# HpWang-whu/RoReg

Measured on AMD Instinct MI355X. Metric: pair-registrations/sec, higher is better.
Workload: dtype f32 (every f32 operand enters the fp16 matrix cores as hi + lo fp16 under a per-keypoint power-of-two block scale: <= 22 significant bits relative to a CONSERVATIVE per-keypoint bound -- measured on the extractor: the bound sits 2^2..2^6 above the keypoint's true coefficient maximum (config.f16x2_sc

## Files before the change

include/roreg_hip.h:

```cpp
#ifndef ROREG_HIP_H
#define ROREG_HIP_H

#include <stdint.h>
#include <stddef.h>

#ifdef __cplusplus
extern "C" {
#endif

#define ROREG_ABI_VERSION 6
int roreg_abi_version(void);
const char *roreg_last_error(void);

int roreg_set_group_tables(const int32_t *P_host, const int32_t *Nei_host, const double *R_host);

size_t roreg_group_conv_packed_size(int Cin, int Cout, int KS);
int roreg_group_conv_pack_weights(const float *W_host , int Cin, int Cout, int KS,
                                  float *wpack_host );
size_t roreg_group_conv_workspace_size(int B, int Cin, int Cout, int Lin, int Lout, int KS);
int roreg_group_conv(const float *x, const float *wpack, const float *bias,
                     const float *bn_scale, const float *bn_shift, const float *residual,
                     float *out, const int32_t *gather,
                     int B, int Cin, int Cout, int Lin, int Lout, int KS,
                     float *workspace, size_t workspace_floats, void *stream);
// ... 186 lines not shown
int roreg_sinkhorn_batch2(const float *src_final, const float *tgt_final, const int32_t *seg_src, const int32_t *seg_tgt,
                          const int32_t *seg_src_host, const int32_t *seg_tgt_host, const float *consts, int n_seg, float alpha, int iters,
                          int64_t *matches0, int64_t *matches1, float *mscores0, float *mscores1, float *ws, size_t ws_floats,
                          int recompute, void *stream);
size_t roreg_sinkhorn_batch3_workspace_size(int n_seg, int max_m, int max_n, long long total_m, long long total_n, int recompute, int want_Z);
int roreg_sinkhorn_batch3(const float *src_final, const float *tgt_final, const int32_t *seg_src, const int32_t *seg_tgt,
                          const int32_t *seg_src_host, const int32_t *seg_tgt_host, const float *consts, int n_seg, float alpha, int iters,
                          int64_t *matches0, int64_t *matches1, float *mscores0, float *mscores1, float *ws, size_t ws_floats,
                          int recompute, float *Z_out, void *stream);
int roreg_write_files(const char *const *paths, const void *const *headers, const int32_t *header_len, const void *const *data,
                      const int64_t *nbytes, int n, int n_threads);
int roreg_yohoc_draw_many(const uint32_t *seeds, int n_pairs, const int64_t *anchors, const int64_t *offsets, int max_iter, int max_tries,
                          int64_t *rows_out, int32_t *n_hyp_out, double *giveup_out, int n_threads);
size_t roreg_mlp_head_workspace(int L, int n_seg, int C1);
int roreg_mlp_head(const float *x, const float *pos, const float *table, const int64_t *idx, const float *conf, int m, int k, int L, int Cin,
                   const float *W1, const float *b1, int C1, const float *Wr, const float *br, float *h, float *y, const int32_t *seg_off,
                   int n_seg, int mult, float eps, float *mean_rstd, double *ws, void *stream);
int roreg_sinkhorn_early_exit(int on);
int roreg_sinkhorn_iteration_stats(long long *iterations, long long *pairs, int reset, void *stream);

int roreg_set_fourier_tables(const float *F_host);
size_t roreg_irrep_gemm_tiles(int O, int B, int32_t *tiles_host);
size_t roreg_irrep_gemm_tiles_m(int O, int B, int tile_m , int32_t *tiles_host);
int roreg_irrep_gemm(const float *const *X, float *const *Out, const float *const *Add, const float *const *Wpack, int C, int O, int B,
                     const int32_t *tiles_dev, int n_tiles, void *stream);
int roreg_irrep_gemm_split(const float *const *X, float *const *Out, const float *const *Add, const void *const *Wsplit, int C, int O, int B,
                           const int32_t *tiles_dev, int n_tiles, void *stream);
int roreg_irrep_gemm_f16x2(const float *const *X, float *const *Out, const float *const *Add, const void *const *Wsplit2,
                           const float *x_bound_dev, int w_exp, const float *next_u_dev, const float *next_v_dev, float *out_bound_dev,
                           int C, int O, int B, const int32_t *tiles_dev, int n_tiles,
                           int tile_m ,
                           int x_planes , void *stream);
int roreg_gemm_persistent(int on);
int roreg_row_bound(const void *x_spatial, int x_bf16 , const float *bn_scale, const float *bn_shift,
                    float *bound_out, int B, int C, void *stream);
int roreg_ft_nonlin(const float *Xin , const float *x_spatial, const float *bias,
                    const float *bias2, const float *bn_scale, const float *bn_shift, const float *resid_spatial,
                    float *Xout , float *out_spatial ,
                    const int32_t *g_map ,
                    int Lout , int Lvalid,
                    int B, int C, int split ,
                    const float *out_bound ,
                    float *out_rowmax ,
                    int spatial_bf16 ,
                    int out_planes ,
                    void *stream);
int roreg_ft_nonlin_packed(const float *Xin, const float *bias, const float *bn_scale, const float *bn_shift, uint32_t *out_words,
                           const int32_t *g_map, int Lout, int Lvalid, int B, int C, const float *out_bound, float *raw_col, int raw_g,
                           void *stream);

int roreg_profile_enable(int on);
int roreg_profile_read(int slot, double *total_ms, int *launches);

#ifdef __cplusplus
}
#endif
#endif
```

roreg_amd/_abi.py:

```python
import ctypes
from ctypes import c_int, c_void_p, c_size_t, c_double, c_float, c_char_p

import numpy as np

ABI_VERSION = 6

_P = c_void_p
PROTOTYPES = {
    'roreg_abi_version': (c_int, []),
    'roreg_last_error': (c_char_p, []),
    'roreg_set_group_tables': (c_int, [_P, _P, _P]),
    'roreg_group_conv_packed_size': (c_size_t, [c_int, c_int, c_int]),
    'roreg_group_conv_pack_weights': (c_int, [_P, c_int, c_int, c_int, _P]),
    'roreg_group_conv_workspace_size': (c_size_t, [c_int, c_int, c_int, c_int, c_int, c_int]),
    'roreg_group_conv': (c_int, [_P, _P, _P, _P, _P, _P, _P, _P, c_int, c_int, c_int, c_int, c_int, c_int, _P, c_size_t, _P]),
    'roreg_group_conv_split': (c_int, [_P, _P, _P, _P, _P, _P, _P, _P, c_int, c_int, c_int, c_int, c_int, c_int, c_int, _P]),
    'roreg_group_conv_f16x2': (c_int, [_P, _P, c_int, _P, _P, _P, c_float, c_float, _P, _P, _P, _P, _P, c_int, c_int, c_int, c_int, c_int, c_int, c_int, _P]),
    'roreg_group_conv_f16x2_packed': (c_int, [_P, _P, c_int, _P, _P, _P, _P, _P, _P, c_int, c_int, c_int, c_int, c_int, c_int, c_int, _P]),
    'roreg_dense_f16x2': (c_int, [_P, _P, c_int, _P, _P, _P, c_float, c_float, _P, _P, c_int, _P, _P, c_int, c_int, c_int, _P]),
    'roreg_dense_split': (c_int, [_P, _P, _P, _P, _P, _P, c_int, _P, c_int, c_int, c_int, _P]),
    'roreg_gf_finalize': (c_int, [_P, _P, c_int, _P, c_int, _P]),
    'roreg_det_score': (c_int, [_P, _P, c_int, _P]),
    'roreg_inv_descriptor': (c_int, [_P, c_int, _P, c_int, _P]),
    'roreg_nn_search': (c_int, [_P, _P, c_int, _P, _P, c_int, c_int, _P, _P, _P, _P]),
# ... 18 lines not shown
    'roreg_quat_to_trans': (c_int, [_P, _P, _P, _P, _P, _P, c_int, _P, _P, _P]),
    'roreg_ransac_score': (c_int, [_P, _P, _P, c_int, c_int, _P, _P, c_int, c_double, _P, _P, _P, _P]),
    'roreg_refine': (c_int, [_P, _P, _P, c_int, c_int, _P, c_int, _P, _P, _P, c_double, _P, _P, _P]),
    'roreg_lt_prepare_batch': (c_int, [_P, c_int, c_int, c_int, _P, _P, _P, _P, _P, _P]),
    'roreg_lt_finish_batch': (c_int, [_P, c_int, c_int, _P, _P, _P, _P]),
    'roreg_ransac_batch_workspace': (c_size_t, [c_int, ctypes.c_longlong, c_int]),
    'roreg_ransac_batch': (c_int, [_P, c_int, ctypes.c_longlong, c_int, c_int, c_double, c_int, _P, _P, _P, _P, _P, _P, c_size_t, _P]),
    'roreg_refine_batch': (c_int, [_P, _P, c_int, ctypes.c_longlong, _P, ctypes.c_double, c_int, _P, _P, _P, _P]),
    'roreg_yohoc_draw': (c_int, [_P, ctypes.c_longlong, _P, _P, c_int, c_int, _P, _P, _P, _P]),
    'roreg_gather_rows_batch': (c_int, [_P, c_int, c_int, c_int, _P]),
    'roreg_gather_rows_f64': (c_int, [_P, _P, c_int, c_int, _P, _P]),
    'roreg_group_corr': (c_int, [_P, _P, _P, _P, c_int, c_int, _P, _P, _P]),
    'roreg_topk_dot_workspace_size': (c_size_t, [c_int, c_int, c_int]),
    'roreg_topk_dot': (c_int, [_P, c_int, _P, c_int, c_int, _P, _P, _P, c_size_t, _P, _P, c_int, c_int, c_int, _P]),
    'roreg_context_colmax': (c_int, [_P, c_int, _P, c_int, c_int, _P, _P, _P]),
    'roreg_sinkhorn_batch_workspace_size': (c_size_t, [c_int, c_int, c_int, ctypes.c_longlong, ctypes.c_longlong]),
    'roreg_sinkhorn_batch_consts': (c_int, [_P, _P, c_int, _P]),
    'roreg_sinkhorn_batch': (c_int, [_P, _P, _P, _P, _P, _P, _P, c_int, c_float, c_int, _P, _P, _P, _P, _P, c_size_t, _P]),
    'roreg_sinkhorn_batch2_workspace_size': (c_size_t, [c_int, c_int, c_int, ctypes.c_longlong, ctypes.c_longlong]),
    'roreg_sinkhorn_batch2': (c_int, [_P, _P, _P, _P, _P, _P, _P, c_int, c_float, c_int, _P, _P, _P, _P, _P, c_size_t, c_int, _P]),
    'roreg_sinkhorn_batch3_workspace_size': (c_size_t, [c_int, c_int, c_int, ctypes.c_longlong, ctypes.c_longlong, c_int, c_int]),
    'roreg_sinkhorn_batch3': (c_int, [_P, _P, _P, _P, _P, _P, _P, c_int, c_float, c_int, _P, _P, _P, _P, _P, c_size_t, c_int, _P, _P]),
    'roreg_write_files': (c_int, [_P, _P, _P, _P, _P, c_int, c_int]),
    'roreg_yohoc_draw_many': (c_int, [_P, c_int, _P, _P, c_int, c_int, _P, _P, _P, c_int]),
    'roreg_mlp_head_workspace': (c_size_t, [c_int, c_int, c_int]),
    'roreg_mlp_head': (c_int, [_P, _P, _P, _P, _P, c_int, c_int, c_int, c_int, _P, _P, c_int, _P, _P, _P, _P, _P, c_int, c_int, c_float, _P, _P, _P]),
    'roreg_sinkhorn_early_exit': (c_int, [c_int]),
    'roreg_sinkhorn_iteration_stats': (c_int, [_P, _P, c_int, _P]),
    'roreg_linear': (c_int, [_P, c_int, c_int, _P, _P, c_int, _P, _P]),
    'roreg_linear_mfma': (c_int, [_P, c_int, c_int, _P, _P, c_int, _P, _P]),
    'roreg_linear_path': (c_int, [c_int]),
    'roreg_linear_cat3': (c_int, [_P, _P, _P, _P, c_int, c_int, _P, _P, c_int, _P, _P]),
    'roreg_gemm_persistent': (c_int, [c_int]),
    'roreg_instnorm_stats': (c_int, [_P, c_int, c_int, c_float, _P, _P, _P, c_int, c_int, _P]),
    'roreg_mlp_tail': (c_int, [_P, c_int, c_int, _P, _P, _P, _P, _P, c_int, c_int, _P]),
    'roreg_mlp_tail_mfma': (c_int, [_P, c_int, c_int, _P, _P, _P, _P, _P, c_int, c_int, _P]),
    'roreg_knn_attention': (c_int, [_P, _P, _P, _P, c_int, c_int, c_int, c_int, _P, _P]),
    'roreg_rm_elementwise': (c_int, [c_int, _P, _P, _P, _P, c_int, c_int, c_int, _P, _P, _P]),
    'roreg_sinkhorn_workspace_size': (c_size_t, [c_int, c_int]),
    'roreg_sinkhorn': (c_int, [_P, c_int, _P, c_int, c_float, c_int, _P, _P, _P, _P, _P, _P, c_size_t, _P]),
    'roreg_profile_enable': (c_int, [c_int]),
    'roreg_profile_read': (c_int, [c_int, _P, _P]),
    'roreg_set_fourier_tables': (c_int, [_P]),
    'roreg_mt_shuffle_prefix': (c_int, [_P, c_int, _P, c_int, c_int, _P, c_int]),
    'roreg_mt_stream_shuffle_prefix': (c_int, [_P, _P, _P, c_int, c_int, _P]),
    'roreg_irrep_gemm_tiles': (c_size_t, [c_int, c_int, _P]),
    'roreg_irrep_gemm_tiles_m': (c_size_t, [c_int, c_int, c_int, _P]),
    'roreg_irrep_gemm': (c_int, [_P, _P, _P, _P, c_int, c_int, c_int, _P, c_int, _P]),
    'roreg_irrep_gemm_split': (c_int, [_P, _P, _P, _P, c_int, c_int, c_int, _P, c_int, _P]),
    'roreg_irrep_gemm_f16x2': (c_int, [_P, _P, _P, _P, _P, c_int, _P, _P, _P, c_int, c_int, c_int, _P, c_int, c_int, c_int, _P]),
    'roreg_row_bound': (c_int, [_P, c_int, _P, _P, _P, c_int, c_int, _P]),
    'roreg_ft_nonlin': (c_int, [_P, _P, _P, _P, _P, _P, _P, _P, _P, _P, c_int, c_int, c_int, c_int, c_int, _P, _P, c_int, c_int, _P]),
    'roreg_ft_nonlin_packed': (c_int, [_P, _P, _P, _P, _P, _P, c_int, c_int, c_int, c_int, _P, _P, c_int, _P]),
}


_RANSAC_TASK = np.dtype([('keys0', np.uint64), ('keys1', np.uint64), ('matches', np.uint64), ('w', np.uint64), ('Trans', np.uint64),
                         ('hyp_rows', np.uint64), ('M', np.int32), ('H', np.int32), ('koff', np.int64)])

_MATCH_TASK = np.dtype([('desc0', np.uint64), ('desc1', np.uint64), ('rows0', np.uint64), ('rows1', np.uint64), ('m0', np.int32), ('m1', np.int32)])

_GATHER_TASK = np.dtype([('src', np.uint64), ('rows', np.uint64), ('dst', np.uint64), ('n', np.int32), ('pad', np.int32)])

_LT_TASK = np.dtype([('before0', np.uint64), ('before1', np.uint64), ('after0', np.uint64), ('after1', np.uint64), ('keys0', np.uint64),
                     ('keys1', np.uint64), ('matches', np.uint64), ('sel', np.uint64), ('n', np.int32), ('pad', np.int32), ('off', np.int64),
                     ('coef0', np.uint64), ('coef1', np.uint64)])
# ... 1 lines not shown
```

roreg_amd/_hip_fourier.py:

```python
import os
from ctypes import c_void_p

import numpy as np
import torch

from . import hip as _core
from .hip import HipError, _check, _feat, _ptr, _stream, lib

__all__ = ['DenseSplitLayer', 'IRREP_DIMS', 'IRREP_OFFSETS', '_bf16_split3', '_keypoint_of_columns', '_ptr_array', '_res_ptr', '_tile_cache', 'bf16_split3_pack', 'bound_exp', 'coef_pitch', 'coef_size', 'coef_views', 'dense_split', 'ensure_fourier', 'f16_scale_exp', 'f16_split2_pack', 'ft_nonlin', 'ft_nonlin_packed', 'gemm_persistent', 'group_conv_split_pack', 'irrep_gemm', 'next_bound', 'next_bound_spatial', 'pack_coefs_f16x2', 'row_bound', 'unpack_coefs_f16x2', 'words_to_planes']


_fourier_ready = False
IRREP_DIMS = (1, 3, 3, 4, 5)
IRREP_OFFSETS = (0, 1, 10, 19, 35, 60)


def ensure_fourier():
    global _fourier_ready
    if not _fourier_ready:
        from .fourier import group_fourier
        F = np.ascontiguousarray(group_fourier().F, np.float32)
        _check(lib().roreg_set_fourier_tables(F.ctypes.data), 'roreg_set_fourier_tables')
        _fourier_ready = True


def _ptr_array(views):
    arr = (c_void_p * 5)(*[c_void_p(v.data_ptr()) for v in views])
    return arr


def coef_pitch(B):
    return (int(B) + 31) // 32 * 32


def coef_size(C, B):
    return 60 * C * coef_pitch(B)


def coef_views(buf, C, B):
    Bp = coef_pitch(B)
    return [buf[IRREP_OFFSETS[r] * C * Bp:IRREP_OFFSETS[r + 1] * C * Bp].view(IRREP_DIMS[r] * C, IRREP_DIMS[r] * Bp) for r in range(5)]

# ... 27 lines not shown
        nu = nv = None
        if next_bound is not None:
            nu, nv = next_bound
            if nu.numel() != O or nv.numel() != O:
                raise HipError('irrep_gemm: next_bound must hold one (u, v) per output channel')
            bound_out = torch.zeros(Bp, dtype=torch.float32, device=X_buf.device)
        _check(lib().roreg_irrep_gemm_f16x2(_ptr_array(xv), _ptr_array(ov), av, _ptr_array(wl), _ptr(x_bound, torch.float32), int(w_exp),
                                            _ptr(nu, torch.float32), _ptr(nv, torch.float32), _ptr(bound_out), C, O, Bp,
                                            _ptr(t, torch.int32), int(t.shape[0]), tile_m, (int(x_planes) if x_planes in (1, 2) and x_planes is not True else (2 if _core.MFMA16 else 1)) if x_planes else 0, _stream()), 'roreg_irrep_gemm_f16x2')
    elif split is not None:
        _check(lib().roreg_irrep_gemm_split(_ptr_array(xv), _ptr_array(ov), av, _ptr_array(split), C, O, Bp, _ptr(t, torch.int32), int(t.shape[0]),
                                            _stream()), 'roreg_irrep_gemm_split')
    else:
        _check(lib().roreg_irrep_gemm(_ptr_array(xv), _ptr_array(ov), av, _ptr_array(Wpacks), C, O, Bp, _ptr(t, torch.int32), int(t.shape[0]), _stream()),
               'roreg_irrep_gemm')
    if _core.PROFILE is not None:
        e1.record(); _core.PROFILE.append((('irrep_gemm_f16x2' if f16x2 is not None else 'irrep_gemm_split' if split is not None else 'irrep_gemm', Bp, C, O), e0, e1))
    return (out, bound_out) if next_bound is not None else out


class gemm_persistent:

    def __init__(self, on=True):
        self.on = int(on)

    def __enter__(self):
        self.prev = lib().roreg_gemm_persistent(self.on)

    def __exit__(self, *exc):
        lib().roreg_gemm_persistent(self.prev)
        return False


def row_bound(x, bn=None):
    B, C = int(x.shape[0]), int(x.shape[1])
    out = torch.empty(coef_pitch(B), dtype=torch.float32, device=x.device)
    scale, shift = bn if bn is not None else (None, None)
    xp, bf = _feat(x)
    _check(lib().roreg_row_bound(xp, bf, _ptr(scale), _ptr(shift), _ptr(out), B, C, _stream()), 'roreg_row_bound')
    return out


def _keypoint_of_columns(d, Bp):
    n = torch.arange(d * Bp, device='cuda')
    return ((n // 32) // d) * 32 + (n % 32)


def bound_exp(bound):
    _, ex = torch.frexp(bound.float())
    e = torch.where((bound > 0) & torch.isfinite(bound), 14 - ex, torch.zeros_like(ex))
    return e.clamp(-100, 100)


def pack_coefs_f16x2(X_buf, C, B, bound=None):
    Bp = coef_pitch(B)
    views = coef_views(X_buf, C, B)
    if bound is None:
        bound = torch.zeros(Bp, dtype=torch.float32, device=X_buf.device)
        for r, v in enumerate(views):
            kp = _keypoint_of_columns(IRREP_DIMS[r], Bp)
            bound.scatter_reduce_(0, kp, v.abs().amax(0), 'amax')
    e = bound_exp(bound)
    out = torch.empty_like(X_buf)
    for r, (v, o) in enumerate(zip(views, coef_views(out, C, B))):
        kp = _keypoint_of_columns(IRREP_DIMS[r], Bp)
        y = torch.ldexp(v, e[kp][None, :])
# ... 183 lines not shown
```

roreg_amd/csrc/fourier.hip:

```cpp
#include "common.h"
#include <algorithm>
#include <atomic>
#include <cmath>
#include <cstdlib>
#include <type_traits>
#include <utility>
#include <vector>

typedef float f32x16 __attribute__((ext_vector_type(16)));

namespace {

constexpr int NIRR = 5;

struct GemmDescs {
    const float *X[NIRR];
    float *Out[NIRR];
    const float *Add[NIRR];
    const float4 *W[NIRR];
    int K[NIRR], M[NIRR], Mpad[NIRR], N[NIRR];
};

inline int round_up(int a, int b) { return (a + b - 1) / b * b; }

// ... 1316 lines not shown
    int kind[32];
    int d[32];
    int row_alpha[16], row_d[16];
};
constexpr PairSlots make_pair_slots() {
    PairSlots t{};
    const int dims[NIRR] = {1, 3, 3, 4, 5};
    int off = 0, s = 0, row0 = 0;
    for (int r = 0; r < NIRR; ++r) {
        const int d = dims[r];
        for (int l = 0; l < d; ++l) {
            t.row_alpha[row0 + l] = off + l * d; t.row_d[row0 + l] = d;
            for (int i = d % 2; i < d; i += 2, ++s) {
                t.qa[s] = off + i * d + l; t.qb[s] = off + (i + 1) * d + l; t.row[s] = row0 + l; t.i[s] = i; t.kind[s] = 0; t.d[s] = d;
            }
        }
        if (d % 2)
            for (int l = 0; l < d; l += 2, ++s) {
                t.qa[s] = off + l; t.row[s] = row0 + l; t.i[s] = 0; t.d[s] = d;
                if (l + 1 < d) { t.qb[s] = off + l + 1; t.kind[s] = 1; } else { t.qb[s] = 64; t.kind[s] = 2; }
            }
        off += d * d; row0 += d;
    }
    return t;
}
constexpr PairSlots kPS = make_pair_slots();
constexpr int slot_out_q(int m) { const int mm = m & 31, s = (m >> 5) * 16 + (mm & 3) + 4 * (mm >> 3); return (mm & 4) ? kPS.qb[s] : kPS.qa[s]; }

template <int... I, class F>
__device__ __forceinline__ void static_for_impl(std::integer_sequence<int, I...>, F &&f) { (f(std::integral_constant<int, I>{}), ...); }
template <int N, class F>
__device__ __forceinline__ void static_for(F &&f) { static_for_impl(std::make_integer_sequence<int, N>{}, f); }

template <bool IN_SPATIAL, bool OUT_SPATIAL, int SPLIT , int NW , int MINW , bool OUT_ROWS = false>
__global__ __launch_bounds__(NW * 64, MINW) void ft_nonlin_kernel(NonlinParams p) {
    constexpr int NT = NW * 64;
    const int lane = threadIdx.x & 63;
    const int jn = lane & 31, h = lane >> 5;
    const int wave_global = __builtin_amdgcn_readfirstlane((blockIdx.x * NT + threadIdx.x) >> 6);
    const int n_waves = gridDim.x * NW;
    const int B = p.B, C = p.C;
    const int n_tiles = C * p.tiles_per_c;

    constexpr int NPL = SPLIT == 2 ? 2 : 3;
    constexpr int NA1 = SPLIT ? 4 * 2 * NPL * 64 * 4 : 30 * 2 * 64, NA2 = SPLIT ? 4 * 2 * NPL * 64 * 4 : 32 * 2 * 64;
    __shared__ __attribute__((aligned(16))) float sA1[IN_SPATIAL ? 64 : NA1];
    __shared__ __attribute__((aligned(16))) float sA2[OUT_SPATIAL ? 64 : NA2];
    __shared__ float sT[(IN_SPATIAL || OUT_SPATIAL || OUT_ROWS) ? NW * 32 * 65 : 64];
    {
        const float *g1 = SPLIT == 3 ? reinterpret_cast<const float *>(p.A1s) : SPLIT == 2 ? reinterpret_cast<const float *>(p.A1h) : p.A1;
        const float *g2 = SPLIT == 3 ? reinterpret_cast<const float *>(p.A2s) : SPLIT == 2 ? reinterpret_cast<const float *>(p.A2h) : p.A2;
        if (!IN_SPATIAL)
            for (int i = threadIdx.x; i < NA1; i += NT) sA1[i] = g1[i];
        if (!OUT_SPATIAL)
            for (int i = threadIdx.x; i < NA2; i += NT) sA2[i] = g2[i];
    }
    __shared__ float sBias[512], sScale[512], sShift[512];
    __shared__ int sGmap[64];
    if (threadIdx.x < 64) sGmap[threadIdx.x] = (OUT_SPATIAL && p.g_map && threadIdx.x < ROREG_G) ? p.g_map[threadIdx.x] : (int)threadIdx.x;
    for (int i = threadIdx.x; i < p.C; i += NT) {
        sBias[i] = (p.bias ? p.bias[i] : 0.f) + (p.bias2 ? p.bias2[i] : 0.f);
        sScale[i] = p.bn_scale ? p.bn_scale[i] : 1.f;
        sShift[i] = p.bn_shift ? p.bn_shift[i] : 0.f;
    }
    __syncthreads();
    const bf16x8 *sA1s = reinterpret_cast<const bf16x8 *>(sA1), *sA2s = reinterpret_cast<const bf16x8 *>(sA2);
    const f16x8 *sA1h = reinterpret_cast<const f16x8 *>(sA1), *sA2h = reinterpret_cast<const f16x8 *>(sA2);
    const size_t Bp = (size_t)p.Bp;
    const size_t hmask = (size_t)0 - (size_t)h;
#define OFF_Q(Q, c, tb) ((size_t)(kQ.alpha[Q] * C + (c) * kQ.d[Q]) * Bp + (size_t)(tb) * (32 * kQ.d[Q]) + kQ.i[Q] * 32)
#define OFF_OF(Q0, Q1, c, tb) (OFF_Q(Q0, c, tb) + ((OFF_Q(Q1, c, tb) - OFF_Q(Q0, c, tb)) & hmask))
    const unsigned lane_next = (unsigned)lane * 4u;
    const unsigned lane_row3 = (unsigned)jn * 4u + (h ? 12u * (unsigned)C * (unsigned)p.Bp : 0u);
    const unsigned lane_row5 = (unsigned)jn * 4u + (h ? 20u * (unsigned)C * (unsigned)p.Bp : 0u);
    auto row_off = [&](auto rc, int c, int tb) -> size_t {
        constexpr int R = decltype(rc)::value;
        return ((size_t)(kPS.row_alpha[R] * C) + (size_t)(c * kPS.row_d[R])) * Bp + (size_t)tb * (32 * kPS.row_d[R]);
    };
    auto slot_ptr = [&](auto sc, const void *buf, int c, int tb) -> const char * {
        constexpr int S = decltype(sc)::value;
        const char *rb = reinterpret_cast<const char *>(buf) + 4 * row_off(std::integral_constant<int, kPS.row[S]>{}, c, tb) + 128 * kPS.i[S];
        return rb + (kPS.kind[S] == 1 ? (kPS.d[S] == 3 ? lane_row3 : lane_row5) : lane_next);
    };

    constexpr int NCV = IN_SPATIAL ? 32 : (SPLIT != 0 ? 32 : 30);
    constexpr bool PACK_OUT = SPLIT == 2 && !OUT_SPATIAL && !OUT_ROWS;
    auto ld_sp = [&](const float *base, size_t i) -> float {
        return p.x_bf16 ? __uint_as_float((unsigned)reinterpret_cast<const unsigned short *>(base)[i] << 16) : base[i];
    };
    float cn[NCV + 1];
// ... 102 lines not shown
                float mx = 0.f;
#pragma unroll
                for (int s = 0; s < 32; ++s) mx = fmaxf(mx, ((16 * (s >> 3) + 8 + (s & 7) < ROREG_G || h == 0) ? fabsf(cv[s]) : 0.f));
                float xsc, osc;
                column_scale(mx, xsc, osc);
#pragma unroll
                for (int st = 0; st < 4; ++st) {
                    float x8[8];
#pragma unroll
                    for (int e = 0; e < 8; ++e) x8[e] = (16 * st + 8 + e < ROREG_G || h == 0) ? cv[st * 8 + e] : 0.f;
                    f16x8 bh, bl;
                    split2(x8, xsc, bh, bl);
                    v[0] = mfma3(sA1h + ((st * 2 + 0) * 2) * 64 + lane, bh, bl, v[0]);
                    v[1] = mfma3(sA1h + ((st * 2 + 1) * 2) * 64 + lane, bh, bl, v[1]);
                }
#pragma unroll
                for (int t = 0; t < 2; ++t)
#pragma unroll
                    for (int r = 0; r < 16; ++r) v[t][r] *= osc;
            } else {
#pragma unroll
                for (int s = 0; s < 30; ++s) {
                    v[0] = __builtin_amdgcn_mfma_f32_32x32x2f32(sA1[(s * 2 + 0) * 64 + lane], cv[s], v[0], 0, 0, 0);
                    v[1] = __builtin_amdgcn_mfma_f32_32x32x2f32(sA1[(s * 2 + 1) * 64 + lane], cv[s], v[1], 0, 0, 0);
                }
            }
        }
        const float bsum = sBias[c];
        const bool bn = p.bn_scale != nullptr;
        const float sc = sScale[c], sh = sShift[c];
        const bool has_rs = OUT_SPATIAL && p.r_spatial;
        const bool rs_late = has_rs && !bn && !p.g_map && !p.out_rowmax;
        const size_t rs = ((size_t)bb * C + c) * ROREG_G;
        float *tb = (OUT_SPATIAL || OUT_ROWS) ? sT + (threadIdx.x >> 6) * (32 * 65) : nullptr;
        const bool sp_pack = OUT_SPATIAL && SPLIT == 2 && p.sp_pack;
        const float pk_scale = sp_pack ? ldexpf(1.f, bound_exp(cv[NCV])) : 1.f;
#pragma unroll
        for (int t = 0; t < 2; ++t)
#pragma unroll
            for (int r = 0; r < 16; ++r) {
                const int g = t * 32 + (r & 3) + 8 * (r >> 2) + 4 * h;
                float x = v[t][r] + bsum;
                if (OUT_SPATIAL && has_rs && !rs_late && g < ROREG_G) x += ld_sp(p.r_spatial, rs + g);
                if (sp_pack && p.raw_col && g == p.raw_g && valid) p.raw_col[(size_t)bb * C + c] = x;
                if (bn) x = fmaxf(fmaf(x, sc, sh), 0.f);
                if (g >= ROREG_G || !valid) x = 0.f;
                v[t][r] = x;
                if (OUT_SPATIAL && g < ROREG_G) {
                    const int go = sGmap[g];
                    if (go >= 0) {
                        if (sp_pack) {
                            const float xs = x * pk_scale;
                            const _Float16 h1 = (_Float16)xs;
                            const _Float16 l1 = (_Float16)(xs - (float)h1);
                            tb[jn * 65 + go] = __uint_as_float((unsigned)__builtin_bit_cast(unsigned short, h1) | ((unsigned)__builtin_bit_cast(unsigned short, l1) << 16));
                        } else {
                            tb[jn * 65 + go] = x; wmax = fmaxf(wmax, fabsf(x));
                        }
                    }
                }
            }
        if (OUT_SPATIAL) {
            asm volatile("s_waitcnt lgkmcnt(0)" ::: "memory");
            const int b0 = tbi * 32;
            if (b0 + 32 <= B) {
                float *ob = p.out_spatial + ((size_t)b0 * C + c) * p.Lout + lane;
                const size_t ostep = (size_t)C * p.Lout;
                const size_t rb = ((size_t)b0 * C + c) * ROREG_G + (lane < ROREG_G ? lane : 0), rstep = (size_t)C * ROREG_G;
                const unsigned short *r16 = reinterpret_cast<const unsigned short *>(p.r_spatial);
#pragma unroll
                for (int g8 = 0; g8 < 4; ++g8) {
                    float tv[8], rv[8];
#pragma unroll
                    for (int q = 0; q < 8; ++q) tv[q] = tb[(g8 * 8 + q) * 65 + lane];
                    if (rs_late) {
                        if (p.x_bf16) {
#pragma unroll
                            for (int q = 0; q < 8; ++q) rv[q] = __uint_as_float((unsigned)r16[rb + (size_t)(g8 * 8 + q) * rstep]);
#pragma unroll
                            for (int q = 0; q < 8; ++q) tv[q] += __uint_as_float(__float_as_uint(rv[q]) << 16);
                        } else {
#pragma unroll
                            for (int q = 0; q < 8; ++q) rv[q] = p.r_spatial[rb + (size_t)(g8 * 8 + q) * rstep];
#pragma unroll
                            for (int q = 0; q < 8; ++q) tv[q] += rv[q];
                        }
                    }
#pragma unroll
                    for (int q = 0; q < 8; ++q)
                        if (lane < p.Lout) ob[(size_t)(g8 * 8 + q) * ostep] = lane < p.Lvalid ? tv[q] : 0.f;
                }
            } else {
                for (int bl = 0; bl < 32 && b0 + bl < B; ++bl)
                    if (lane < p.Lout) {
                        float tv = tb[bl * 65 + lane];
// ... 87 lines not shown
                        float tv[8];
#pragma unroll
                        for (int q = 0; q < 8; ++q) tv[q] = tb[(g8 * 8 + q) * 65 + lane];
#pragma unroll
                        for (int q = 0; q < 8; ++q)
                            if (lane < ROREG_G) ob[(size_t)(g8 * 8 + q) * ostep] = tv[q];
                    }
                } else {
                    for (int bl = 0; bl < 32 && b0 + bl < B; ++bl)
                        if (lane < ROREG_G) p.out_spatial[((size_t)(b0 + bl) * C + c) * ROREG_G + lane] = tb[bl * 65 + lane];
                }
                asm volatile("s_waitcnt lgkmcnt(0)" ::: "memory");
            } else if (PACK_OUT && p.out_planes) {
                const int tb = tbi;
                const unsigned sel = (jn & 16) ? 0x07060302u : 0x05040100u;
                static_for<32>([&](auto ic) {
                    constexpr int S = decltype(ic)::value, t = S / 16, r = S % 16;
                    const unsigned own = __float_as_uint(o[t][r]);
                    const auto pr = __builtin_amdgcn_permlane16_swap(own, own, false, false);
                    const unsigned word = __builtin_amdgcn_perm(pr[1], pr[0], sel);
                    unsigned *dst = reinterpret_cast<unsigned *>(const_cast<char *>(slot_ptr(ic, p.Xout, c, tb)));
                    if (kPS.kind[S] != 2 || h == 0) __builtin_nontemporal_store(word, dst);
                });
            } else {
                const int tb = tbi;
                static_for<32>([&](auto ic) {
                    constexpr int S = decltype(ic)::value, t = S / 16, r = S % 16;
                    float *dst = reinterpret_cast<float *>(const_cast<char *>(slot_ptr(ic, p.Xout, c, tb)));
                    if (kPS.kind[S] != 2 || h == 0) __builtin_nontemporal_store(o[t][r], dst);
                });
            }
        }
    };
    if (wave_global < n_tiles) {
        const int last = wave_global + ((n_tiles - 1 - wave_global) / n_waves) * n_waves;
        float cb[NCV + 1];
        load_coefs(wave_global, cn);
        __builtin_amdgcn_s_waitcnt(0x0F70);
        for (int tile = wave_global; tile <= last; tile += 2 * n_waves) {
            const int t1 = min(tile + n_waves, last), t2 = min(tile + 2 * n_waves, last);
            process(tile, t1, cn, cb);
            process(t1, t2, cb, cn);
        }
    }
}

#undef OFF_OF
#undef OFF_Q

float *g_A1 = nullptr, *g_A2 = nullptr;
uint16_t *g_A1s = nullptr, *g_A2s = nullptr, *g_A1h = nullptr, *g_A2h = nullptr;
int g_f_exp = 0;

}

extern "C" int roreg_set_fourier_tables(const float *F_host ) {
    ROREG_REQUIRE(F_host, "roreg_set_fourier_tables: null table");
    static float A1[30 * 2 * 64], A2[32 * 2 * 64];
    for (int s = 0; s < 30; ++s)
        for (int tile = 0; tile < 2; ++tile)
            for (int lane = 0; lane < 64; ++lane) {
                const int qq = 2 * s + (lane >> 5), g = tile * 32 + (lane & 31);
                A1[(s * 2 + tile) * 64 + lane] = g < 60 ? F_host[qq * 60 + g] : 0.f;
            }
    for (int t = 0; t < 2; ++t)
        for (int r = 0; r < 16; ++r)
            for (int tile = 0; tile < 2; ++tile)
// ... 134 lines not shown
}

extern "C" int roreg_irrep_gemm(const float *const *X, float *const *Out, const float *const *Add, const float *const *Wpack, int C, int O, int B,
                                const int32_t *tiles_dev, int n_tiles, void *stream) {
    ROREG_REQUIRE(X && Out && Wpack && tiles_dev && C > 0 && O > 0 && B > 0 && n_tiles > 0, "roreg_irrep_gemm: bad arguments");
    ROREG_REQUIRE(C % 32 == 0, "roreg_irrep_gemm: C must be a multiple of 32 (got %d)", C);
    ROREG_REQUIRE(B % 4 == 0, "roreg_irrep_gemm: B must be a multiple of 4 (got %d); pad the keypoint batch", B);
    static const int dims[5] = {1, 3, 3, 4, 5};
    GemmDescs p;
    for (int r = 0; r < 5; ++r) {
        p.X[r] = X[r]; p.Out[r] = Out[r]; p.Add[r] = Add ? Add[r] : nullptr; p.W[r] = reinterpret_cast<const float4 *>(Wpack[r]);
        p.K[r] = dims[r] * C; p.M[r] = dims[r] * O; p.Mpad[r] = round_up(dims[r] * O, 128); p.N[r] = dims[r] * B;
    }
    constexpr int CT = 32;
    const size_t lds = 2 * CT * 256 * sizeof(float);
    auto kern = irrep_gemm_kernel<CT>;
    hipError_t e = hipFuncSetAttribute(reinterpret_cast<const void *>(kern), hipFuncAttributeMaxDynamicSharedMemorySize, (int)lds);
    if (e != hipSuccess) { roreg::set_error("roreg_irrep_gemm: hipFuncSetAttribute: %s", hipGetErrorString(e)); return 1; }
    hipLaunchKernelGGL(kern, dim3(n_tiles), dim3(256), lds, roreg::as_stream(stream), p, tiles_dev);
    ROREG_CHECK_LAUNCH("roreg_irrep_gemm");
    return 0;
}

#define ROREG_GEMM_PERSIST_DEFAULT 0
static std::atomic<int> g_gemm_persist{-1};
static int gemm_launch_form() {
    int v = g_gemm_persist.load(std::memory_order_relaxed);
    if (v < 0) {
        const char *e = getenv("ROREG_GEMM_PERSIST");
        v = e ? (e[0] == '1' ? 1 : e[0] == '2' ? 2 : 0) : ROREG_GEMM_PERSIST_DEFAULT;
        g_gemm_persist.store(v, std::memory_order_relaxed);
    }
    return v;
}
extern "C" int roreg_gemm_persistent(int on) {
    const int prev = gemm_launch_form();
    if (on >= 0 && on <= 2) g_gemm_persist.store(on, std::memory_order_relaxed);
    return prev;
}
static int gemm_cu_count() {
    static const int n = [] {
        int dev = 0, cus = 0;
        if (hipGetDevice(&dev) != hipSuccess || hipDeviceGetAttribute(&cus, hipDeviceAttributeMultiprocessorCount, dev) != hipSuccess || cus <= 0) cus = 256;
        return cus;
    }();
    return n;
}
template <int NP, int WO>
static int launch_gemm_split(const char *what, const float *const *X, float *const *Out, const float *const *Add, const void *const *Wsplit,
                             const float *xbound, int w_exp, const float *nb_u, const float *nb_v, float *out_bound, int C, int O, int B,
                             const int32_t *tiles_dev, int n_tiles, void *stream, int x_planes = 0) {
    static const int dims[5] = {1, 3, 3, 4, 5};
    GemmSplitDescs p;
    for (int r = 0; r < 5; ++r) {
        p.X[r] = X[r]; p.Out[r] = Out[r]; p.Add[r] = Add ? Add[r] : nullptr; p.W[r] = Wsplit[r];
        p.K[r] = dims[r] * C; p.M[r] = dims[r] * O; p.Mpad[r] = round_up(dims[r] * O, 128); p.N[r] = dims[r] * B;
        if (WO == 4 && p.Mpad[r] % 256 != 0) { roreg::set_error("%s: tile_m = 256 needs O %% 256 == 0 (got %d)", what, O); return 2; }
    }
    p.xbound = xbound; p.w_exp = w_exp; p.nb_u = nb_u; p.nb_v = nb_v; p.out_bound = out_bound; p.O = O;
    constexpr int CT = 32;
    const size_t lds = 2 * (NP * 2 * 256 + NP * (WO * 64) * 2) * 16;
    if (x_planes) {
        if constexpr (NP == 2 && WO == 4) {
            const size_t lds_x = 3 * (2 * 16 * 256 * 2) + 2 * (2 * 2 * 256) * 16;
            const bool mfma16 = x_planes == 2;
            const size_t lds_use = mfma16 ? (size_t)(6 + 4) * 16384 : lds_x;
// ... 106 lines not shown

extern "C" int roreg_ft_nonlin(const float *Xin, const float *x_spatial, const float *bias, const float *bias2,
                               const float *bn_scale, const float *bn_shift, const float *resid_spatial, float *Xout, float *out_spatial,
                               const int32_t *g_map, int Lout, int Lvalid, int B, int C, int split, const float *out_bound, float *out_rowmax,
                               int spatial_bf16, int out_planes, void *stream) {
    ROREG_REQUIRE(g_A1 && g_A2, "roreg_ft_nonlin: roreg_set_fourier_tables has not been called");
    ROREG_REQUIRE((Xin != nullptr) != (x_spatial != nullptr), "roreg_ft_nonlin: exactly one of Xin / x_spatial");
    ROREG_REQUIRE((Xout != nullptr) != (out_spatial != nullptr), "roreg_ft_nonlin: exactly one of Xout / out_spatial");
    ROREG_REQUIRE((bn_scale == nullptr) == (bn_shift == nullptr) && B > 0 && C > 0 && C <= 512, "roreg_ft_nonlin: bad arguments (C <= 512)");
    ROREG_REQUIRE((long long)60 * C * B < (1ll << 40), "roreg_ft_nonlin: tensor too large");
    ROREG_REQUIRE(!g_map || (Lout >= Lvalid && Lvalid > 0 && Lout <= 64), "roreg_ft_nonlin: bad Lout/Lvalid");
    NonlinParams p;
    memset(&p, 0, sizeof(p));
    p.Xin = Xin; p.Xout = Xout;
    p.x_spatial = x_spatial; p.r_spatial = resid_spatial; p.out_spatial = out_spatial;
    p.g_map = g_map; p.Lout = g_map ? Lout : ROREG_G; p.Lvalid = g_map ? Lvalid : ROREG_G;
    p.bias = bias; p.bias2 = bias2; p.bn_scale = bn_scale; p.bn_shift = bn_shift; p.A1 = g_A1; p.A2 = g_A2;
    p.A1s = reinterpret_cast<const bf16x8 *>(g_A1s); p.A2s = reinterpret_cast<const bf16x8 *>(g_A2s); p.out_bound = out_bound; p.out_rowmax = out_rowmax; p.x_bf16 = spatial_bf16;
    p.A1h = reinterpret_cast<const f16x8 *>(g_A1h); p.A2h = reinterpret_cast<const f16x8 *>(g_A2h); p.f_exp = g_f_exp;
    p.B = B; p.Bp = (B + 31) / 32 * 32; p.C = C; p.tiles_per_c = (B + 31) / 32;
    p.out_planes = out_planes;
    ROREG_REQUIRE((unsigned long long)C * p.Bp * 20ull < (1ull << 32), "roreg_ft_nonlin: C * round_up(B, 32) must stay below 2^32 / 20 (32-bit lane offsets)");
    ROREG_REQUIRE(!out_planes || (split == 2 && Xout), "roreg_ft_nonlin: out_planes is a layout of the fp16 x 2 coefficient output");
    const long long n_tiles = (long long)C * p.tiles_per_c;
    hipStream_t s = roreg::as_stream(stream);
    roreg::ProfScope prof(roreg::PROF_FT_NONLIN, s);
    const bool in_sp = x_spatial != nullptr, out_sp = out_spatial != nullptr;
    if (in_sp && out_sp) { roreg::set_error("roreg_ft_nonlin: spatial -> spatial is not a transform"); return 2; }
    ROREG_REQUIRE(split != 2 || out_sp || out_bound, "roreg_ft_nonlin: split = 2 writes the coefficients as fp16 hi/lo pairs and needs out_bound");
    ROREG_REQUIRE(!spatial_bf16 || in_sp || resid_spatial, "roreg_ft_nonlin: spatial_bf16 refers to x_spatial / resid_spatial");
    ROREG_REQUIRE(!out_rowmax || out_sp, "roreg_ft_nonlin: out_rowmax goes with a group-domain output");
    ROREG_REQUIRE(split >= 0 && split <= 2, "roreg_ft_nonlin: split must be 0 (f32 MFMA), 1 (bf16 x 3) or 2 (fp16 x 2)");
    if (split == 2) {
        if (in_sp) launch_ft<ft_nonlin_kernel<true, false, 2, 4, 1>>(p, n_tiles, s);
        else if (!out_sp) launch_ft<ft_nonlin_kernel<false, false, 2, 4, 1>>(p, n_tiles, s);
        else launch_ft<ft_nonlin_kernel<false, true, 2, 4, 1>>(p, n_tiles, s);
    } else if (split == 1) {
        if (in_sp) launch_ft<ft_nonlin_kernel<true, false, 3, 4, 1>>(p, n_tiles, s);
        else if (!out_sp) launch_ft<ft_nonlin_kernel<false, false, 3, 4, 1>>(p, n_tiles, s);
        else launch_ft<ft_nonlin_kernel<false, true, 3, 4, 1>>(p, n_tiles, s);
    } else {
        if (in_sp) launch_ft<ft_nonlin_kernel<true, false, 0, 4, 1>>(p, n_tiles, s);
        else if (!out_sp) launch_ft<ft_nonlin_kernel<false, false, 0, 4, 1>>(p, n_tiles, s);
        else launch_ft<ft_nonlin_kernel<false, true, 0, 4, 1>>(p, n_tiles, s);
    }
    ROREG_CHECK_LAUNCH("roreg_ft_nonlin");
    return 0;
}

extern "C" int roreg_ft_nonlin_packed(const float *Xin, const float *bias, const float *bn_scale, const float *bn_shift, uint32_t *out_words,
                                      const int32_t *g_map, int Lout, int Lvalid, int B, int C, const float *out_bound, float *raw_col, int raw_g,
                                      void *stream) {
    ROREG_REQUIRE(g_A1 && g_A2, "roreg_ft_nonlin_packed: roreg_set_fourier_tables has not been called");
    ROREG_REQUIRE(Xin && out_words && out_bound && B > 0 && C > 0 && C <= 512 && (bn_scale == nullptr) == (bn_shift == nullptr), "roreg_ft_nonlin_packed: bad arguments");
    ROREG_REQUIRE(!g_map || (Lout >= Lvalid && Lvalid > 0 && Lout <= 64), "roreg_ft_nonlin_packed: bad Lout/Lvalid");
    ROREG_REQUIRE(!raw_col || (raw_g >= 0 && raw_g < ROREG_G), "roreg_ft_nonlin_packed: raw_g out of range");
    NonlinParams p;
    memset(&p, 0, sizeof(p));
    p.Xin = Xin; p.out_spatial = reinterpret_cast<float *>(out_words);
    p.g_map = g_map; p.Lout = g_map ? Lout : ROREG_G; p.Lvalid = g_map ? Lvalid : ROREG_G;
    p.bias = bias; p.bn_scale = bn_scale; p.bn_shift = bn_shift; p.A1 = g_A1; p.A2 = g_A2;
    p.A1s = reinterpret_cast<const bf16x8 *>(g_A1s); p.A2s = reinterpret_cast<const bf16x8 *>(g_A2s);
    p.A1h = reinterpret_cast<const f16x8 *>(g_A1h); p.A2h = reinterpret_cast<const f16x8 *>(g_A2h); p.f_exp = g_f_exp;
    p.out_bound = out_bound; p.sp_pack = 1; p.raw_col = raw_col; p.raw_g = raw_g;
    p.B = B; p.Bp = (B + 31) / 32 * 32; p.C = C; p.tiles_per_c = (B + 31) / 32;
    ROREG_REQUIRE((unsigned long long)C * p.Bp * 20ull < (1ull << 32), "roreg_ft_nonlin_packed: C * round_up(B, 32) must stay below 2^32 / 20 (32-bit lane offsets)");
    hipStream_t s = roreg::as_stream(stream);
    roreg::ProfScope prof(roreg::PROF_FT_NONLIN, s);
    launch_ft<ft_nonlin_kernel<false, true, 2, 4, 1>>(p, (long long)C * p.tiles_per_c, s);
    ROREG_CHECK_LAUNCH("roreg_ft_nonlin_packed");
    return 0;
}

extern "C" int roreg_feat_coefs(const void *x, int x_bf16, float *out, int B, int C, int split, void *stream) {
    if (B == 0) return 0;
    ROREG_REQUIRE(g_A1 && g_A2, "roreg_feat_coefs: roreg_set_fourier_tables has not been called");
    ROREG_REQUIRE(x && out && B > 0 && C > 0 && C <= 512 && split >= 0 && split <= 2, "roreg_feat_coefs: bad arguments");
    NonlinParams p;
    memset(&p, 0, sizeof(p));
    p.x_spatial = reinterpret_cast<const float *>(x); p.x_bf16 = x_bf16; p.out_spatial = out;
    p.Lout = ROREG_G; p.Lvalid = ROREG_G; p.A1 = g_A1; p.A2 = g_A2;
    p.A1s = reinterpret_cast<const bf16x8 *>(g_A1s); p.A2s = reinterpret_cast<const bf16x8 *>(g_A2s);
    p.A1h = reinterpret_cast<const f16x8 *>(g_A1h); p.A2h = reinterpret_cast<const f16x8 *>(g_A2h); p.f_exp = g_f_exp;
    p.B = B; p.Bp = (B + 31) / 32 * 32; p.C = C; p.tiles_per_c = (B + 31) / 32;
    const long long n_tiles = (long long)C * p.tiles_per_c;
    hipStream_t s = roreg::as_stream(stream);
    if (split == 2) launch_ft<ft_nonlin_kernel<true, false, 2, 4, 1, true>>(p, n_tiles, s);
    else if (split == 1) launch_ft<ft_nonlin_kernel<true, false, 3, 4, 1, true>>(p, n_tiles, s);
    else launch_ft<ft_nonlin_kernel<true, false, 0, 4, 1, true>>(p, n_tiles, s);
    ROREG_CHECK_LAUNCH("roreg_feat_coefs");
    return 0;
}
```

Measured before the change: 1101.

## Add thin ft_nonlin kernel variants with higher occupancy and wide packed-output staging

Adds a runtime switch, on by default, that selects ft_nonlin kernel instantiations with a 256-channel shared table and launch bounds requesting three blocks per CU, so that more waves can be resident when C <= 256. For the packed group-domain output it adds a WIDE mode. In this mode four waves each handle one channel of the same 32-row batch tile and stage into a shared tile of width 4*Lout. After a block barrier the tile is written to global memory as contiguous rows, and raw_col goes through shared memory. The aim is to coalesce global stores and raise occupancy. The cost is two block-wide barriers per round and extra shared-memory zeroing.

```diff
diff --git a/include/roreg_hip.h b/include/roreg_hip.h
--- a/include/roreg_hip.h
+++ b/include/roreg_hip.h
@@ -242,6 +242,7 @@
                            int tile_m ,
                            int x_planes , void *stream);
 int roreg_gemm_persistent(int on);
+int roreg_thin_kernels(int on);
 int roreg_row_bound(const void *x_spatial, int x_bf16 , const float *bn_scale, const float *bn_shift,
                     float *bound_out, int B, int C, void *stream);
 int roreg_ft_nonlin(const float *Xin , const float *x_spatial, const float *bias,
diff --git a/roreg_amd/_abi.py b/roreg_amd/_abi.py
--- a/roreg_amd/_abi.py
+++ b/roreg_amd/_abi.py
@@ -74,6 +74,7 @@
     'roreg_linear_path': (c_int, [c_int]),
     'roreg_linear_cat3': (c_int, [_P, _P, _P, _P, c_int, c_int, _P, _P, c_int, _P, _P]),
     'roreg_gemm_persistent': (c_int, [c_int]),
+    'roreg_thin_kernels': (c_int, [c_int]),
     'roreg_instnorm_stats': (c_int, [_P, c_int, c_int, c_float, _P, _P, _P, c_int, c_int, _P]),
     'roreg_mlp_tail': (c_int, [_P, c_int, c_int, _P, _P, _P, _P, _P, c_int, c_int, _P]),
     'roreg_mlp_tail_mfma': (c_int, [_P, c_int, c_int, _P, _P, _P, _P, _P, c_int, c_int, _P]),
diff --git a/roreg_amd/_hip_fourier.py b/roreg_amd/_hip_fourier.py
--- a/roreg_amd/_hip_fourier.py
+++ b/roreg_amd/_hip_fourier.py
@@ -7,7 +7,7 @@
 from . import hip as _core
 from .hip import HipError, _check, _feat, _ptr, _stream, lib
 
-__all__ = ['DenseSplitLayer', 'IRREP_DIMS', 'IRREP_OFFSETS', '_bf16_split3', '_keypoint_of_columns', '_ptr_array', '_res_ptr', '_tile_cache', 'bf16_split3_pack', 'bound_exp', 'coef_pitch', 'coef_size', 'coef_views', 'dense_split', 'ensure_fourier', 'f16_scale_exp', 'f16_split2_pack', 'ft_nonlin', 'ft_nonlin_packed', 'gemm_persistent', 'group_conv_split_pack', 'irrep_gemm', 'next_bound', 'next_bound_spatial', 'pack_coefs_f16x2', 'row_bound', 'unpack_coefs_f16x2', 'words_to_planes']
+__all__ = ['DenseSplitLayer', 'IRREP_DIMS', 'IRREP_OFFSETS', '_bf16_split3', '_keypoint_of_columns', '_ptr_array', '_res_ptr', '_tile_cache', 'bf16_split3_pack', 'bound_exp', 'coef_pitch', 'coef_size', 'coef_views', 'dense_split', 'ensure_fourier', 'f16_scale_exp', 'f16_split2_pack', 'ft_nonlin', 'ft_nonlin_packed', 'gemm_persistent', 'group_conv_split_pack', 'irrep_gemm', 'next_bound', 'next_bound_spatial', 'pack_coefs_f16x2', 'row_bound', 'thin_kernels', 'unpack_coefs_f16x2', 'words_to_planes']
 
 
 _fourier_ready = False
@@ -101,6 +101,19 @@
         return False
 
 
+class thin_kernels:
+
+    def __init__(self, on=True):
+        self.on = int(bool(on))
+
+    def __enter__(self):
+        self.prev = lib().roreg_thin_kernels(self.on)
+
+    def __exit__(self, *exc):
+        lib().roreg_thin_kernels(self.prev)
+        return False
+
+
 def row_bound(x, bn=None):
     B, C = int(x.shape[0]), int(x.shape[1])
     out = torch.empty(coef_pitch(B), dtype=torch.float32, device=x.device)
diff --git a/roreg_amd/csrc/fourier.hip b/roreg_amd/csrc/fourier.hip
--- a/roreg_amd/csrc/fourier.hip
+++ b/roreg_amd/csrc/fourier.hip
@@ -1372,8 +1372,10 @@
 template <int N, class F>
 __device__ __forceinline__ void static_for(F &&f) { static_for_impl(std::make_integer_sequence<int, N>{}, f); }
 
-template <bool IN_SPATIAL, bool OUT_SPATIAL, int SPLIT , int NW , int MINW , bool OUT_ROWS = false>
+constexpr int WIDE_NCH = 4, WIDE_LOUT_MAX = 48;
+template <bool IN_SPATIAL, bool OUT_SPATIAL, int SPLIT , int NW , int MINW , bool OUT_ROWS = false, bool WIDE = false, int CMAX = 512 >
 __global__ __launch_bounds__(NW * 64, MINW) void ft_nonlin_kernel(NonlinParams p) {
+    static_assert(!WIDE || (OUT_SPATIAL && !IN_SPATIAL && SPLIT == 2 && WIDE_NCH == NW), "WIDE: the packed group-domain output, one channel per wave and round");
     constexpr int NT = NW * 64;
     const int lane = threadIdx.x & 63;
     const int jn = lane & 31, h = lane >> 5;
@@ -1386,7 +1388,11 @@
     constexpr int NA1 = SPLIT ? 4 * 2 * NPL * 64 * 4 : 30 * 2 * 64, NA2 = SPLIT ? 4 * 2 * NPL * 64 * 4 : 32 * 2 * 64;
     __shared__ __attribute__((aligned(16))) float sA1[IN_SPATIAL ? 64 : NA1];
     __shared__ __attribute__((aligned(16))) float sA2[OUT_SPATIAL ? 64 : NA2];
-    __shared__ float sT[(IN_SPATIAL || OUT_SPATIAL || OUT_ROWS) ? NW * 32 * 65 : 64];
+    __shared__ float sT[WIDE ? 32 * (WIDE_NCH * WIDE_LOUT_MAX + 1) : (IN_SPATIAL || OUT_SPATIAL || OUT_ROWS) ? NW * 32 * 65 : 64];
+    __shared__ float sRaw[WIDE ? 32 * (WIDE_NCH + 1) : 1];
+    const int wide_w = WIDE_NCH * p.Lout, wide_pitch = wide_w | 1;
+    if constexpr (WIDE)
+        for (int i = threadIdx.x; i < 32 * (WIDE_NCH * WIDE_LOUT_MAX + 1); i += NT) sT[i] = 0.f;
     {
         const float *g1 = SPLIT == 3 ? reinterpret_cast<const float *>(p.A1s) : SPLIT == 2 ? reinterpret_cast<const float *>(p.A1h) : p.A1;
         const float *g2 = SPLIT == 3 ? reinterpret_cast<const float *>(p.A2s) : SPLIT == 2 ? reinterpret_cast<const float *>(p.A2h) : p.A2;
@@ -1395,7 +1401,7 @@
         if (!OUT_SPATIAL)
             for (int i = threadIdx.x; i < NA2; i += NT) sA2[i] = g2[i];
     }
-    __shared__ float sBias[512], sScale[512], sShift[512];
+    __shared__ float sBias[CMAX], sScale[CMAX], sShift[CMAX];
     __shared__ int sGmap[64];
     if (threadIdx.x < 64) sGmap[threadIdx.x] = (OUT_SPATIAL && p.g_map && threadIdx.x < ROREG_G) ? p.g_map[threadIdx.x] : (int)threadIdx.x;
     for (int i = threadIdx.x; i < p.C; i += NT) {
@@ -1564,7 +1570,8 @@
         const bool has_rs = OUT_SPATIAL && p.r_spatial;
         const bool rs_late = has_rs && !bn && !p.g_map && !p.out_rowmax;
         const size_t rs = ((size_t)bb * C + c) * ROREG_G;
-        float *tb = (OUT_SPATIAL || OUT_ROWS) ? sT + (threadIdx.x >> 6) * (32 * 65) : nullptr;
+        float *tb = WIDE ? sT + (c % WIDE_NCH) * p.Lout : (OUT_SPATIAL || OUT_ROWS) ? sT + (threadIdx.x >> 6) * (32 * 65) : nullptr;
+        const int tpitch = WIDE ? wide_pitch : 65;
         const bool sp_pack = OUT_SPATIAL && SPLIT == 2 && p.sp_pack;
         const float pk_scale = sp_pack ? ldexpf(1.f, bound_exp(cv[NCV])) : 1.f;
 #pragma unroll
@@ -1574,25 +1581,26 @@
                 const int g = t * 32 + (r & 3) + 8 * (r >> 2) + 4 * h;
                 float x = v[t][r] + bsum;
                 if (OUT_SPATIAL && has_rs && !rs_late && g < ROREG_G) x += ld_sp(p.r_spatial, rs + g);
-                if (sp_pack && p.raw_col && g == p.raw_g && valid) p.raw_col[(size_t)bb * C + c] = x;
+                if constexpr (WIDE) { if (g == p.raw_g) sRaw[jn * (WIDE_NCH + 1) + c % WIDE_NCH] = x; }
+                else if (sp_pack && p.raw_col && g == p.raw_g && valid) p.raw_col[(size_t)bb * C + c] = x;
                 if (bn) x = fmaxf(fmaf(x, sc, sh), 0.f);
                 if (g >= ROREG_G || !valid) x = 0.f;
                 v[t][r] = x;
                 if (OUT_SPATIAL && g < ROREG_G) {
                     const int go = sGmap[g];
-                    if (go >= 0) {
+                    if (go >= 0 && (!WIDE || go < p.Lvalid)) {
                         if (sp_pack) {
                             const float xs = x * pk_scale;
                             const _Float16 h1 = (_Float16)xs;
                             const _Float16 l1 = (_Float16)(xs - (float)h1);
-                            tb[jn * 65 + go] = __uint_as_float((unsigned)__builtin_bit_cast(unsigned short, h1) | ((unsigned)__builtin_bit_cast(unsigned short, l1) << 16));
+                            tb[jn * tpitch + go] = __uint_as_float((unsigned)__builtin_bit_cast(unsigned short, h1) | ((unsigned)__builtin_bit_cast(unsigned short, l1) << 16));
                         } else {
-                            tb[jn * 65 + go] = x; wmax = fmaxf(wmax, fabsf(x));
+                            tb[jn * tpitch + go] = x; wmax = fmaxf(wmax, fabsf(x));
                         }
                     }
                 }
             }
-        if (OUT_SPATIAL) {
+        if (OUT_SPATIAL && !WIDE) {
             asm volatile("s_waitcnt lgkmcnt(0)" ::: "memory");
             const int b0 = tbi * 32;
             if (b0 + 32 <= B) {
@@ -1746,7 +1754,51 @@
             }
         }
     };
-    if (wave_global < n_tiles) {
+    if constexpr (WIDE) {
+        const int wv = __builtin_amdgcn_readfirstlane((int)(threadIdx.x >> 6));
+        const int runs = C / WIDE_NCH, n_rounds = p.tiles_per_c * runs, G = (int)gridDim.x;
+        auto tile_of = [&](int r) { const int tbr = r / runs; return tbr * C + (r - tbr * runs) * WIDE_NCH + wv; };
+        auto flush = [&](int r) {
+            asm volatile("s_waitcnt lgkmcnt(0)\n\ts_barrier" ::: "memory");
+            const int tbr = r / runs, c0 = (r - tbr * runs) * WIDE_NCH, b0 = tbr * 32;
+            const int nrow = B - b0 < 32 ? B - b0 : 32;
+            float *ob = p.out_spatial + ((size_t)b0 * C + c0) * p.Lout + lane;
+            const size_t ostep = (size_t)C * p.Lout;
+            constexpr int NJ = (WIDE_NCH * WIDE_LOUT_MAX + 63) / 64;
+            const int nj = (wide_w + 63) >> 6;
+#pragma unroll
+            for (int rr = 0; rr < 32 / NW; ++rr) {
+                const int row = rr * NW + wv;
+                if (row < nrow) {
+                    float tv[NJ];
+#pragma unroll
+                    for (int j = 0; j < NJ; ++j)
+                        if (j < nj) tv[j] = sT[row * wide_pitch + (lane + 64 * j < wide_w ? lane + 64 * j : 0)];
+#pragma unroll
+                    for (int j = 0; j < NJ; ++j)
+                        if (j < nj && lane + 64 * j < wide_w) ob[(size_t)row * ostep + 64 * j] = tv[j];
+                }
+            }
+            if (p.raw_col && threadIdx.x < 32 * WIDE_NCH) {
+                const int row = threadIdx.x / WIDE_NCH, cc = threadIdx.x % WIDE_NCH;
+                if (row < nrow) p.raw_col[(size_t)(b0 + row) * C + c0 + cc] = sRaw[row * (WIDE_NCH + 1) + cc];
+            }
+            asm volatile("s_waitcnt lgkmcnt(0)\n\ts_barrier" ::: "memory");
+        };
+        if ((int)blockIdx.x < n_rounds) {
+            const int first = blockIdx.x, last = first + ((n_rounds - 1 - first) / G) * G;
+            float cb[NCV + 1];
+            load_coefs(tile_of(first), cn);
+            __builtin_amdgcn_s_waitcnt(0x0F70);
+            for (int r = first; r <= last; r += 2 * G) {
+                const int r1 = min(r + G, last), r2 = min(r + 2 * G, last);
+                process(tile_of(r), tile_of(r1), cn, cb);
+                flush(r);
+                process(tile_of(r1), tile_of(r2), cb, cn);
+                flush(r1);
+            }
+        }
+    } else if (wave_global < n_tiles) {
         const int last = wave_global + ((n_tiles - 1 - wave_global) / n_waves) * n_waves;
         float cb[NCV + 1];
         load_coefs(wave_global, cn);
@@ -1947,6 +1999,13 @@
         g_gemm_persist.store(v, std::memory_order_relaxed);
     }
     return v;
+}
+static std::atomic<int> g_thin_kernels{1};
+static bool thin_kernels_on() { return g_thin_kernels.load(std::memory_order_relaxed) != 0; }
+extern "C" int roreg_thin_kernels(int on) {
+    const int prev = g_thin_kernels.load(std::memory_order_relaxed);
+    if (on == 0 || on == 1) g_thin_kernels.store(on, std::memory_order_relaxed);
+    return prev;
 }
 extern "C" int roreg_gemm_persistent(int on) {
     const int prev = gemm_launch_form();
@@ -2119,8 +2178,10 @@
     ROREG_REQUIRE(!out_rowmax || out_sp, "roreg_ft_nonlin: out_rowmax goes with a group-domain output");
     ROREG_REQUIRE(split >= 0 && split <= 2, "roreg_ft_nonlin: split must be 0 (f32 MFMA), 1 (bf16 x 3) or 2 (fp16 x 2)");
     if (split == 2) {
-        if (in_sp) launch_ft<ft_nonlin_kernel<true, false, 2, 4, 1>>(p, n_tiles, s);
+        const bool three = thin_kernels_on() && C <= 256;
+        if (in_sp) { if (three) launch_ft<ft_nonlin_kernel<true, false, 2, 4, 3, false, false, 256>>(p, n_tiles, s); else launch_ft<ft_nonlin_kernel<true, false, 2, 4, 1>>(p, n_tiles, s); }
         else if (!out_sp) launch_ft<ft_nonlin_kernel<false, false, 2, 4, 1>>(p, n_tiles, s);
+        else if (three) launch_ft<ft_nonlin_kernel<false, true, 2, 4, 3, false, false, 256>>(p, n_tiles, s);
         else launch_ft<ft_nonlin_kernel<false, true, 2, 4, 1>>(p, n_tiles, s);
     } else if (split == 1) {
         if (in_sp) launch_ft<ft_nonlin_kernel<true, false, 3, 4, 1>>(p, n_tiles, s);
@@ -2154,7 +2215,8 @@
     ROREG_REQUIRE((unsigned long long)C * p.Bp * 20ull < (1ull << 32), "roreg_ft_nonlin_packed: C * round_up(B, 32) must stay below 2^32 / 20 (32-bit lane offsets)");
     hipStream_t s = roreg::as_stream(stream);
     roreg::ProfScope prof(roreg::PROF_FT_NONLIN, s);
-    launch_ft<ft_nonlin_kernel<false, true, 2, 4, 1>>(p, (long long)C * p.tiles_per_c, s);
+    if (thin_kernels_on() && C % WIDE_NCH == 0 && C <= 256 && p.Lout <= WIDE_LOUT_MAX) launch_ft<ft_nonlin_kernel<false, true, 2, 4, 3, false, true, 256>>(p, (long long)(C / WIDE_NCH) * p.tiles_per_c * 4, s);
+    else launch_ft<ft_nonlin_kernel<false, true, 2, 4, 1>>(p, (long long)C * p.tiles_per_c, s);
     ROREG_CHECK_LAUNCH("roreg_ft_nonlin_packed");
     return 0;
 }
@@ -2172,7 +2234,8 @@
     p.B = B; p.Bp = (B + 31) / 32 * 32; p.C = C; p.tiles_per_c = (B + 31) / 32;
     const long long n_tiles = (long long)C * p.tiles_per_c;
     hipStream_t s = roreg::as_stream(stream);
-    if (split == 2) launch_ft<ft_nonlin_kernel<true, false, 2, 4, 1, true>>(p, n_tiles, s);
+    if (split == 2 && thin_kernels_on() && C <= 256) launch_ft<ft_nonlin_kernel<true, false, 2, 4, 3, true, false, 256>>(p, n_tiles, s);
+    else if (split == 2) launch_ft<ft_nonlin_kernel<true, false, 2, 4, 1, true>>(p, n_tiles, s);
     else if (split == 1) launch_ft<ft_nonlin_kernel<true, false, 3, 4, 1, true>>(p, n_tiles, s);
     else launch_ft<ft_nonlin_kernel<true, false, 0, 4, 1, true>>(p, n_tiles, s);
     ROREG_CHECK_LAUNCH("roreg_feat_coefs");
```

After: 1112, median of 6. 1.1% higher.
